# AndyWu0719/Audio-CALM

Measured on NVIDIA B200. Metric: log-mel audio-hours/sec, higher is better.
Workload: dtype f32

## Files before the change

### audio-calm_b200/csrc/acb_kernels.cu

```cuda
#include "audiocalm_b200.h"
#include "acb_fft32.cuh"

#include <cuda_bf16.h>
#include <cuda_runtime.h>

#include <algorithm>
#include <cmath>
#include <cstdio>
#include <cstring>
#include <mutex>
#include <numeric>
#include <string>
#include <vector>

#if !defined(ACB_DEV) || !defined(ACB_ABLATE)
#undef ACB_ABLATE
#define ACB_ABLATE 0
#endif

#ifndef ACB_WIN_FUSE
#define ACB_WIN_FUSE 1
#endif
#ifndef ACB_WIN_T
#define ACB_WIN_T 1
// ... 18 lines not shown
constexpr int kMaxWeights = 4096;
constexpr int kOutStageOffset = 2 * kBins;
static_assert(kScratchFloats % 32 == 8 && kScratchFloats % 4 == 0, "pair stride must be 8 (mod 32) words and 16-byte aligned");
static_assert(kOutStageOffset + kTileFrames * (kMaxMels | 1) <= kScratchFloats, "staged tile must fit above the power spectrum");

thread_local std::string g_last_error;

int fail(int code, const std::string& msg) {
    g_last_error = msg;
    return code;
}
static int cuda_fail(cudaError_t e, const char* what) {
    g_last_error = std::string(what) + ": " + cudaGetErrorString(e);
    return ACB_ERR_CUDA;
}
#define ACB_CUDA(call)                                  \
    do {                                                \
        cudaError_t e__ = (call);                       \
        if (e__ != cudaSuccess) return cuda_fail(e__, #call); \
    } while (0)

__device__ __forceinline__ unsigned smem_addr(const void* p) { return static_cast<unsigned>(__cvta_generic_to_shared(p)); }
__device__ __forceinline__ void mbar_init(unsigned long long* bar, unsigned count) {
    asm volatile("mbarrier.init.shared::cta.b64 [%0], %1;" ::"r"(smem_addr(bar)), "r"(count) : "memory");
}
__device__ __forceinline__ void mbar_arrive(unsigned long long* bar) {
    asm volatile("mbarrier.arrive.shared::cta.b64 _, [%0];" ::"r"(smem_addr(bar)) : "memory");
}
__device__ __forceinline__ void mbar_arrive_expect_tx(unsigned long long* bar, unsigned bytes) {
    asm volatile("mbarrier.arrive.expect_tx.shared::cta.b64 _, [%0], %1;" ::"r"(smem_addr(bar)), "r"(bytes) : "memory");
}
__device__ __forceinline__ bool mbar_wait(unsigned long long* bar, unsigned parity) {
    unsigned ok = 0;
    for (int spin = 0; spin < (1 << 26) && !ok; ++spin) {
        asm volatile("{\n\t.reg .pred p;\n\tmbarrier.try_wait.parity.shared::cta.b64 p, [%1], %2;\n\tselp.u32 %0, 1, 0, p;\n\t}\n"
                     : "=r"(ok) : "r"(smem_addr(bar)), "r"(parity) : "memory");
    }
    return ok != 0;
}
__device__ __forceinline__ void bulk_copy_g2s(void* smem, const void* gmem, unsigned bytes, unsigned long long* bar) {
    asm volatile("cp.async.bulk.shared::cluster.global.mbarrier::complete_tx::bytes [%0], [%1], %2, [%3];"
                 ::"r"(smem_addr(smem)), "l"(gmem), "r"(bytes), "r"(smem_addr(bar)) : "memory");
}

struct LogmelParams {
    const float* window;
    const float4* twiddle;
    const float* plan_w;
    const int* plan_woff;
    const short* plan_trip;
    const short* plan_band;
    const short* plan_astart;
    int n_plan_w;
    int n_mels;
    float clamp_min;
    float log_scale;
    float log_floor;
    const float* wav;
    const long long* clip_offset;
    const long long* clip_length;
    long long clip_stride;
    long long uniform_length;
    const int* tile_start;
    int n_clips;
    int n_tiles;
    int uniform_tiles_per_clip;
    const float* clip_peak;
    void* out;
    int out_bf16;
    int time_major;
    const long long* out_offset;
    long long out_clip_stride;
    long long frame_capacity;
    const long long* frame_capacity_per_clip;
    int pad_multiple;
    int fill_tail;
    float fill_value;
    int affine;
    float affine_mean;
    float affine_inv_std;
    const float* bin_mean;
    const float* bin_std;
    double* moments_partial;
    int* error_flag;
};

struct SmemLayout {
    int samples, scratch, twiddle, window, plan_w, affine, plan_rec, mbar, moments, total_bytes;
};

__host__ __device__ inline int out_row_stride(int n_mels) { return n_mels | 1; }

__host__ __device__ inline SmemLayout make_smem_layout(int kGroups, int n_mels, int n_plan_w, bool with_moments = false) {
    SmemLayout L;
    int off = 0;
    L.samples = off; off += kGroups * kTileSamples;
    L.scratch = off; off += kGroups * kGroupWarps * kScratchFloats;
    L.twiddle = off; off += 5 * 32 * 4;
    L.window = off; off += 32 * 20;
    if (!with_moments) {
        L.plan_rec = off; off += kGroupWarps * kMaxRounds * kSlots * 4;
        L.mbar = off; off += 2 * kGroups;
        off = (off + 3) & ~3;
        L.affine = off; off += 2 * kMaxMels;
        L.plan_w = off; off += (n_plan_w + 3) & ~3;
        L.moments = off;
// ... 194 lines not shown
        const int lane = tid & 31, warp = tid >> 5;
        for (int b = warp; b < n_mels; b += kGroupWarps) fill_span<OutT>(out + (size_t)b * c.cap + f_begin, n_fill, fv, lane, 32);
    }
}

__device__ __forceinline__ float lg2_normal(float x) {
    float y;
    asm("lg2.approx.ftz.f32 %0, %1;" : "=f"(y) : "f"(x));
    return y;
}

__device__ __forceinline__ void two_sum_add(float2& acc, float x) {
    const float t = __fadd_rn(acc.x, x);
    const float bb = __fsub_rn(t, acc.x);
    const float e = __fadd_rn(__fsub_rn(acc.x, __fsub_rn(t, bb)), __fsub_rn(x, bb));
    acc.y = __fadd_rn(acc.y, e);
    acc.x = t;
}

template <int G, bool kMoments, typename OutT>
__global__ void __launch_bounds__(G * kGroupThreads, G == 4 ? 1 : 2) logmel_fused_kernel(const LogmelParams p) {
    constexpr int kGroups = G;
    constexpr int kThreads = G * kGroupThreads;
    extern __shared__ __align__(16) float smem[];
    const SmemLayout L = make_smem_layout(G, p.n_mels, p.n_plan_w, kMoments);
    const int tid = threadIdx.x;
    const int lane = tid & 31;
    const int grp = tid / kGroupThreads;
    const int gt = tid % kGroupThreads;
    const int gw = gt >> 5;
    const int n_mels = p.n_mels;
    const int S = out_row_stride(n_mels);
    const bool write_out = p.out != nullptr;

    float* s_samples = smem + L.samples + grp * kTileSamples;
    float* s_scratch = smem + L.scratch + grp * kGroupWarps * kScratchFloats;
    float* s_out = s_scratch + kOutStageOffset;
    float4* s_tw4 = reinterpret_cast<float4*>(smem + L.twiddle);
    float* s_win = smem + L.window;
    float* s_pw = smem + L.plan_w;
    float2* s_aff = reinterpret_cast<float2*>(smem + L.affine);
    int4* s_rec = reinterpret_cast<int4*>(smem + L.plan_rec);
    float2* s_mom = reinterpret_cast<float2*>(smem + L.moments) + grp * 2 * n_mels;
    unsigned long long* s_full = reinterpret_cast<unsigned long long*>(smem + L.mbar) + grp;

    for (int i = tid; i < 5 * 32; i += kThreads) s_tw4[i] = p.twiddle[i];
    for (int i = tid; i < kNfft / 2; i += kThreads) {
        if (ACB_WIN_T) s_win[(i & 31) * 20 + (i >> 5)] = p.window[i];
        else s_win[i] = p.window[i];
    }
    for (int i = tid; i < p.n_plan_w; i += kThreads) s_pw[i] = p.plan_w[i];
    for (int i = tid; i < kGroupWarps * kMaxRounds * kSlots; i += kThreads) {
        const int slot = i / kSlots, qq = i - slot * kSlots;
        s_rec[i] = make_int4(p.plan_astart[i] >> 1, (p.plan_woff[slot] >> 1) + qq, p.plan_band[i], p.plan_trip[slot]);
    }
    for (int i = tid; i < n_mels; i += kThreads) {
        float sc = 1.f, sh = 0.f;
        if (p.affine == 1) { sc = p.affine_inv_std; sh = -p.affine_mean * p.affine_inv_std; }
        else if (p.affine == 2) { sc = 1.f / __ldg(p.bin_std + i); sh = -__ldg(p.bin_mean + i) * sc; }
        s_aff[i] = make_float2(sc, sh);
    }
    if (kMoments)
        for (int i = gt; i < 2 * n_mels; i += kGroupThreads) s_mom[i] = make_float2(0.f, 0.f);
    if (gt == 0) {
        mbar_init(s_full, 1);
        asm volatile("fence.mbarrier_init.release.cluster;" ::: "memory");
    }
    __syncthreads();

    const long long n_groups = (long long)gridDim.x * kGroups, g_index = (long long)blockIdx.x * kGroups + grp;
    const long long t_begin = (long long)p.n_tiles * g_index / n_groups;
    const long long t_end = (long long)p.n_tiles * (g_index + 1) / n_groups;

    ClipCursor cur;
    bool staged = false;
    unsigned full_parity = 0;
    if (t_begin < t_end) {
        cursor_init(p, cur, t_begin);
        staged = cur.tile_in_clip * kTileFrames < cur.frames;
        if (staged) load_tile_samples(p, cur, s_samples, gt, grp, s_full);
    }

    const int q = lane >> 2;
    const int pl = lane & 3;
    const float* pair_scratch = s_scratch + pl * kScratchFloats;
    float* scr = s_scratch + gw * kScratchFloats;
    float2* scr2 = reinterpret_cast<float2*>(scr);

    for (long long tile = t_begin; tile < t_end; ++tile) {
        if (staged) {
            if (!mbar_wait(s_full, full_parity) && lane == 0) atomicExch(p.error_flag, 1);
            full_parity ^= 1;
        }

        const int f0 = cur.tile_in_clip * kTileFrames;
        const bool has_frames = f0 < cur.frames;
        const bool active = has_frames && f0 + 2 * gw < cur.frames && ACB_ABLATE != 7;

        if (active) {
            float2 pr[16], pi[16];
            {
                const float* sp = s_samples + (2 * gw) * kHop + lane;
                float2 v[20];
#pragma unroll
                for (int r = 0; r < 20; ++r) v[r] = make_float2(sp[32 * (2 * r)], sp[32 * (2 * r + 1)]);
                float4 w4[4];
                if (ACB_WIN_T) {
// ... 56 lines not shown
            __syncwarp();
            {
                const float4* re4 = reinterpret_cast<const float4*>(scr + lane * kRowStride);
                const float4* im4 = reinterpret_cast<const float4*>(scr + kPlaneFloats + lane * kRowStride);
#pragma unroll
                for (int h = 0; h < 8; ++h) {
                    const float4 zr = re4[h], zi = im4[h];
                    pr[brev3(h)] = make_float2(zr.x, zr.y);
                    pr[brev3(h) + 8] = make_float2(zr.z, zr.w);
                    pi[brev3(h)] = make_float2(zi.x, zi.y);
                    pi[brev3(h) + 8] = make_float2(zi.z, zi.w);
                }
            }
            __syncwarp();
            fft32_packed(pr, pi);
            const int src_lane = (32 - lane) & 31;
#pragma unroll
            for (int m = 0; m < 16; ++m) {
                const float alt_r = (m == 0) ? pr[0].x : pr[16 - m].y;
                const float alt_i = (m == 0) ? pi[0].x : pi[16 - m].y;
                const float offer_r = (lane == 0) ? alt_r : pr[15 - m].y;
                const float offer_i = (lane == 0) ? alt_i : pi[15 - m].y;
                const float c = __shfl_sync(0xffffffffu, offer_r, src_lane);
                const float d = __shfl_sync(0xffffffffu, offer_i, src_lane);
                const float a = pr[m].x, b = pi[m].x;
                const float apc = a + c, bmd = b - d, amc = a - c, bpd = b + d;
                const float pa = fmaf(apc, apc, bmd * bmd);
                const float pb = fmaf(amc, amc, bpd * bpd);
                scr2[lane + 32 * m] = make_float2(pa, pb);
            }
        }
        else {
            group_sync(grp);
        }
        const int4* my_rec = s_rec + (gw * kMaxRounds) * kSlots + q;
        int4 rec_next = my_rec[0];
        group_sync(grp);

        ClipCursor nxt = cur;
        staged = false;
        if (tile + 1 < t_end) {
            cursor_advance(p, nxt);
            staged = nxt.tile_in_clip * kTileFrames < nxt.frames;
            if (staged) load_tile_samples(p, nxt, s_samples, gt, grp, s_full);
        }

        const int pad = cur.frames_padded - cur.frames;
        const bool direct = !p.time_major && (f0 + kTileFrames - 1 <= cur.frames - 2 - pad);

        if (has_frames && ACB_ABLATE != 8) {
            const int fA = f0 + 2 * pl;
            OutT* out_clip = reinterpret_cast<OutT*>(p.out) + cur.out_base;
            const bool pair_store = ((cur.cap & 1) == 0) && ((reinterpret_cast<uintptr_t>(out_clip) & (2 * sizeof(OutT) - 1)) == 0);
            for (int r = 0; r < kMaxRounds; ++r) {
                const int4 rec = rec_next;
                const int trip = rec.w;
                if (trip == 0) break;
                if (r + 1 < kMaxRounds) rec_next = my_rec[(r + 1) * kSlots];
                const int b = rec.z;
                const float2 af = s_aff[b < 0 ? 0 : b];
                const float4* p4 = reinterpret_cast<const float4*>(pair_scratch) + rec.x;
                const float2* w2 = reinterpret_cast<const float2*>(s_pw) + rec.y;
                float acc0 = 0.f, acc1 = 0.f, acc2 = 0.f, acc3 = 0.f;
                const int half_trip = ACB_ABLATE == 4 ? 0 : (trip >> 1);
#pragma unroll 4
                for (int i = 0; i < half_trip; ++i) {
                    const float4 pw = p4[i];
                    const float2 w = w2[kSlots * i];
                    acc0 = fmaf(w.x, pw.x, acc0);
                    acc1 = fmaf(w.x, pw.y, acc1);
                    acc2 = fmaf(w.y, pw.z, acc2);
                    acc3 = fmaf(w.y, pw.w, acc3);
                }
                const float mA = (acc0 + acc2) * cur.gain, mB = (acc1 + acc3) * cur.gain;
                float vA = (mA > p.clamp_min) ? lg2_normal(mA) * p.log_scale : p.log_floor;
                float vB = (mB > p.clamp_min) ? lg2_normal(mB) * p.log_scale : p.log_floor;
                if (kMoments) {
                    float s = 0.f, s2 = 0.f;
                    if (b >= 0 && fA < cur.frames) {
                        const float c = (fA <= cur.frames - 2 && fA > cur.frames - 2 - pad) ? 2.f : 1.f;
                        s = c * vA;
                        s2 = s * vA;
                    }
                    if (b >= 0 && fA + 1 < cur.frames) {
                        const float c = (fA + 1 <= cur.frames - 2 && fA + 1 > cur.frames - 2 - pad) ? 2.f : 1.f;
                        const float cv = c * vB;
                        s += cv;
                        s2 = fmaf(cv, vB, s2);
                    }
                    const bool upper = (pl & 2) != 0;
                    float keep = (upper ? s2 : s) + __shfl_xor_sync(0xffffffffu, upper ? s : s2, 2);
                    keep += __shfl_xor_sync(0xffffffffu, keep, 1);
                    if ((pl & 1) == 0 && b >= 0)
                        two_sum_add(s_mom[(upper ? n_mels : 0) + b], keep);
                }
                if (b >= 0) {
                    vA = fmaf(vA, af.x, af.y);
                    vB = fmaf(vB, af.x, af.y);
                    if (direct) {
                        if (write_out) {
                            OutT* dst = out_clip + (size_t)((unsigned)b * (unsigned)cur.cap) + fA;
                            if (pair_store) {
                                store_pair<OutT>(dst, vA, vB);
                            } else {
                                dst[0] = to_out<OutT>(vA);
                                dst[1] = to_out<OutT>(vB);
                            }
                        }
                    } else {
                        s_out[(2 * pl) * S + b] = vA;
                        s_out[(2 * pl + 1) * S + b] = vB;
                    }
                }
            }
        }
        if (!direct) {
            group_sync(grp);
            if (write_out) {
                store_tile<OutT>(p, cur, s_out, n_mels, S, gt);
                if (p.fill_tail && p.tile_start != nullptr && cur.tile_in_clip == cur.tiles_in_clip - 1) fill_row_tail<OutT>(p, cur, n_mels, gt);
            }
        }
        cur = nxt;
    }

    if (kMoments) {
        group_sync(grp);
// ... 358 lines not shown
                                                            long long out_frames, float pad_value,
                                                            const long long* __restrict__ mask_start, const long long* __restrict__ mask_len) {
    constexpr int kT = 64;
    __shared__ float tile[kT][kT + 1];
    const int clip = blockIdx.z;
    const long long t0 = (long long)blockIdx.x * kT;
    const int d0 = blockIdx.y * kT;
    const long long n = lens[clip];
    const T* src = feat + row_offset[clip] * dim;
    const long long m0 = mask_start ? mask_start[clip] : 0, m1 = mask_start ? m0 + mask_len[clip] : 0;
    const int q = threadIdx.x & 15, r0 = threadIdx.x >> 4;
    const bool vec_in = sizeof(T) == 4 && (dim & 3) == 0 && (reinterpret_cast<uintptr_t>(src) & 15) == 0;
#pragma unroll
    for (int pass = 0; pass < kT / 16; ++pass) {
        const int r = pass * 16 + r0;
        const long long t = t0 + r;
        const int d = d0 + 4 * q;
        float v[4] = {pad_value, pad_value, pad_value, pad_value};
        if (t < n) {
            const bool masked = t >= m0 && t < m1;
            if (vec_in && d + 3 < dim) {
                if constexpr (sizeof(T) == 4) {
                    const float4 u = __ldg(reinterpret_cast<const float4*>(src + t * dim + d));
                    v[0] = u.x; v[1] = u.y; v[2] = u.z; v[3] = u.w;
                }
            } else {
#pragma unroll
                for (int j = 0; j < 4; ++j) if (d + j < dim) v[j] = (float)src[t * dim + d + j];
            }
            if (masked) { v[0] = v[1] = v[2] = v[3] = 0.f; }
        }
#pragma unroll
        for (int j = 0; j < 4; ++j) tile[4 * q + j][r] = v[j];
    }
    __syncthreads();
    const bool vec_out = sizeof(T) == 4 && (out_frames & 3) == 0 && (reinterpret_cast<uintptr_t>(out) & 15) == 0;
#pragma unroll
    for (int pass = 0; pass < kT / 16; ++pass) {
        const int r = pass * 16 + r0;
        const int d = d0 + r;
        const long long t = t0 + 4 * q;
        if (d >= dim || t >= out_frames) continue;
        T* dst = out + ((long long)clip * dim + d) * out_frames + t;
        if (vec_out && t + 3 < out_frames) {
            if constexpr (sizeof(T) == 4)
                *reinterpret_cast<float4*>(dst) = make_float4(tile[r][4 * q], tile[r][4 * q + 1], tile[r][4 * q + 2], tile[r][4 * q + 3]);
        } else {
#pragma unroll
            for (int j = 0; j < 4; ++j) if (t + j < out_frames) dst[j] = from_float<T>(tile[r][4 * q + j]);
        }
    }
}

}

struct acb_frontend {
    int device = 0;
    int n_fft = 0, hop = 0, n_mels = 0, n_weights = 0, log_kind = 0;
    float clamp_min = 0.f;
    int num_sms = 0;
    int groups = 0;
    int grid = 0;
    int smem_bytes = 0;
    int smem_bytes_moments = 0;
    void* d_blob = nullptr;
    const float* d_window = nullptr;
    const float4* d_twiddle = nullptr;
    const float* d_plan_w = nullptr;
    const int* d_plan_woff = nullptr;
    const short* d_plan_trip = nullptr;
    const short* d_plan_band = nullptr;
    const short* d_plan_astart = nullptr;
    int n_plan_w = 0;
    int* d_err = nullptr;
    cudaStream_t s_in = nullptr, s_out = nullptr;
    std::vector<cudaEvent_t> ev;
    std::mutex mu;
};

using namespace acb;

extern "C" {

int acb_abi_version(void) { return ACB_ABI_VERSION; }
const char* acb_last_error(void) { return g_last_error.c_str(); }
int acb_frames_per_tile(void) { return kTileFrames; }

int64_t acb_frames_for_length(int64_t length, int n_fft, int hop) {
    if (n_fft <= 0 || hop <= 0) return -1;
    if (length <= n_fft / 2) return -1;
    return 1 + length / hop;
}

int64_t acb_padded_frames(int64_t frames, int multiple) {
    if (multiple <= 1) return frames;
    const int64_t r = frames % multiple;
    return r ? frames + (multiple - r) : frames;
}

int64_t acb_plan_tiles(const int64_t* lengths_host, int32_t n_clips, int n_fft, int hop, int64_t frame_capacity,
                       int32_t* tile_start_host) {
    if (!lengths_host || !tile_start_host || n_clips < 0) return fail(ACB_ERR_INVALID, "acb_plan_tiles: null argument");
    int64_t total = 0;
    for (int32_t i = 0; i < n_clips; ++i) {
        const int64_t T = acb_frames_for_length(lengths_host[i], n_fft, hop);
        if (T < 0) {
            return fail(ACB_ERR_INVALID, "acb_plan_tiles: clip " + std::to_string(i) + " has " + std::to_string(lengths_host[i]) +
                                             " samples; reflect padding needs more than " + std::to_string(n_fft / 2));
        }
        const int64_t cover = frame_capacity > 0 ? frame_capacity : T;
        tile_start_host[i] = (int32_t)total;
        total += (cover + kTileFrames - 1) / kTileFrames;
        if (total > INT32_MAX) return fail(ACB_ERR_INVALID, "acb_plan_tiles: more than 2^31 tiles in one call");
    }
    tile_start_host[n_clips] = (int32_t)total;
    return total;
}

int acb_frontend_create(acb_frontend** out, int device, int n_fft, int hop, int n_mels, const float* window_host,
                        const float* fb_host, float clamp_min, int log_kind) {
    if (!out || !window_host || !fb_host) return fail(ACB_ERR_INVALID, "acb_frontend_create: null argument");
    if (n_fft != kNfft || hop != kHop)
        return fail(ACB_ERR_UNSUPPORTED, "acb_frontend_create: this build has kernels for n_fft=1024, hop=256 only (got n_fft=" +
                                             std::to_string(n_fft) + ", hop=" + std::to_string(hop) + ")");
    if (n_mels < 1 || n_mels > kMaxMels) return fail(ACB_ERR_UNSUPPORTED, "acb_frontend_create: n_mels must be in [1, 128]");
    if (log_kind != ACB_LOG_NATURAL && log_kind != ACB_LOG_10) return fail(ACB_ERR_INVALID, "acb_frontend_create: bad log_kind");
    if (!(clamp_min >= 1.17549435e-38f)) return fail(ACB_ERR_INVALID, "acb_frontend_create: clamp_min must be a positive normal float");
    for (int n = 0; n < kNfft / 2; ++n) {
        const double dev = std::fabs((double)window_host[n + kNfft / 2] - (1.0 - (double)window_host[n]));
        if (!(dev <= 1e-6))
            return fail(ACB_ERR_UNSUPPORTED, "acb_frontend_create: the window must have the periodic-Hann property w[n + 512] = 1 - w[n] "
                                             "(deviation " + std::to_string(dev) + " at n=" + std::to_string(n) + ")");
    }
    const int n_freq = n_fft / 2 + 1;

    std::vector<int> start(n_mels, 0), len(n_mels, 0), off(n_mels, 0);
    std::vector<float> weights;
    for (int m = 0; m < n_mels; ++m) {
        int lo = -1, hi = -1;
        for (int f = 0; f < n_freq; ++f)
            if (fb_host[(size_t)f * n_mels + m] != 0.f) { if (lo < 0) lo = f; hi = f; }
        off[m] = (int)weights.size();
        if (lo >= 0) {
            if (hi >= kBins) {
                if (fb_host[(size_t)(n_freq - 1) * n_mels + m] != 0.f)
                    return fail(ACB_ERR_UNSUPPORTED, "acb_frontend_create: filterbank has weight on the Nyquist bin");
            }
            start[m] = lo;
            len[m] = hi - lo + 1;
            for (int f = lo; f <= hi; ++f) weights.push_back(fb_host[(size_t)f * n_mels + m] * 0.25f);
        }
    }
    if ((int)weights.size() > kMaxWeights) return fail(ACB_ERR_UNSUPPORTED, "acb_frontend_create: filterbank too dense");

    std::vector<int> alen(n_mels), aend(n_mels);
    for (int m = 0; m < n_mels; ++m) {
        if (len[m] == 0) { start[m] = 0; len[m] = 0; }
        aend[m] = (start[m] + std::max(len[m], 1) + 1) & ~1;
        alen[m] = aend[m] - (start[m] & ~1);
    }
    std::vector<int> order(n_mels);
    std::iota(order.begin(), order.end(), 0);
    std::stable_sort(order.begin(), order.end(), [&](int a, int b) { return alen[a] > alen[b]; });
    const int n_rounds = (n_mels + kSlots - 1) / kSlots;
    std::vector<short> plan_band(kGroupWarps * kMaxRounds * kSlots, (short)-1), plan_astart(kGroupWarps * kMaxRounds * kSlots, (short)0),
        plan_trip(kGroupWarps * kMaxRounds, (short)0);
    std::vector<int> plan_woff(kGroupWarps * kMaxRounds, 0);
    std::vector<float> plan_w;
    std::vector<int> load(kGroupWarps, 0), rounds(kGroupWarps, 0);
    for (int g = 0; g < n_rounds; ++g) {
        int best = -1;
        for (int w = 0; w < kGroupWarps; ++w)
            if (rounds[w] < kMaxRounds && (best < 0 || load[w] < load[best])) best = w;
        if (best < 0) return fail(ACB_ERR_UNSUPPORTED, "acb_frontend_create: mel plan overflow");
        std::vector<int> par[2];
        for (int q = 0; q < kSlots && kSlots * g + q < n_mels; ++q) {
            const int m = order[kSlots * g + q];
            par[((start[m] & ~1) >> 1) & 1].push_back(m);
        }
        std::vector<int> slots;
        while (!par[0].empty() && !par[1].empty()) {
            slots.push_back(par[0].back()); par[0].pop_back();
            slots.push_back(par[1].back()); par[1].pop_back();
        }
        for (int k = 0; k < 2; ++k)
            for (int m : par[k]) slots.push_back(m);
        std::vector<int> shift(slots.size(), 0), as(slots.size(), 0);
        int trip = 2;
        for (int iter = 0; iter < 8; ++iter) {
            trip = 2;
            for (size_t i = 0; i < slots.size(); ++i) trip = std::max(trip, aend[slots[i]] - ((start[slots[i]] & ~1) - shift[i]));
            for (size_t i = 0; i < slots.size(); ++i) {
                as[i] = (start[slots[i]] & ~1) - shift[i];
                if (as[i] + trip > kBins) as[i] = std::max(0, (kBins - trip) & ~1);
            }
            bool changed = false;
            for (size_t i = 0; i + 1 < slots.size(); i += 2) {
                if ((((as[i] >> 1) ^ (as[i + 1] >> 1)) & 1) != 0) continue;
                const size_t x = (as[i + 1] >= 2 && (start[slots[i + 1]] & ~1) - shift[i + 1] == as[i + 1]) ? i + 1
                                 : ((as[i] >= 2 && (start[slots[i]] & ~1) - shift[i] == as[i]) ? i : slots.size());
                if (x < slots.size()) { shift[x] += 2; changed = true; }
            }
            if (!changed) break;
        }
        const int slot = best * kMaxRounds + rounds[best];
        plan_trip[slot] = (short)trip;
        plan_woff[slot] = (int)plan_w.size();
        plan_w.resize(plan_w.size() + (size_t)trip * kSlots, 0.f);
        float* wbase = plan_w.data() + plan_woff[slot];
        for (size_t q = 0; q < slots.size(); ++q) {
            const int m = slots[q];
            plan_band[slot * kSlots + q] = (short)m;
            plan_astart[slot * kSlots + q] = (short)as[q];
            for (int i = 0; i < len[m]; ++i) {
                const int rel = start[m] + i - as[q];
                if (rel < 0 || rel >= trip) return fail(ACB_ERR_UNSUPPORTED, "acb_frontend_create: mel plan window error");
                wbase[(rel >> 1) * (2 * kSlots) + q * 2 + (rel & 1)] = weights[off[m] + i];
            }
        }
        load[best] += trip + 16;
        rounds[best]++;
    }
    if ((int)plan_w.size() > kMaxWeights * 4) return fail(ACB_ERR_UNSUPPORTED, "acb_frontend_create: mel plan too large");

    std::vector<float4> tw(5 * 32);
    for (int l = 0; l < 32; ++l) {
        auto wre = [&](int m) { return (float)cos(-2.0 * M_PI * (double)(m * l) / 1024.0); };
        auto wim = [&](int m) { return (float)sin(-2.0 * M_PI * (double)(m * l) / 1024.0); };
        for (int k = 0; k < 4; ++k) tw[k * 32 + l] = make_float4(wre(k), wre(k + 16), wim(k), wim(k + 16));
        tw[4 * 32 + l] = make_float4(wre(4), wim(4), 0.f, 0.f);
    }

    int prev = 0;
    ACB_CUDA(cudaGetDevice(&prev));
    ACB_CUDA(cudaSetDevice(device));
    auto* fe = new acb_frontend();
    fe->device = device; fe->n_fft = n_fft; fe->hop = hop; fe->n_mels = n_mels; fe->n_weights = (int)weights.size();
    fe->n_plan_w = (int)plan_w.size();
    fe->log_kind = log_kind; fe->clamp_min = clamp_min;

    size_t o = 0;
    auto take = [&](size_t bytes) { size_t r = o; o += (bytes + 255) & ~size_t(255); return r; };
    const size_t o_win = take(sizeof(float) * kNfft), o_tw = take(sizeof(float4) * 160),
                 o_pw = take(sizeof(float) * std::max<size_t>(plan_w.size(), 1)), o_po = take(sizeof(int) * plan_woff.size()),
                 o_pt = take(sizeof(short) * plan_trip.size()), o_pb = take(sizeof(short) * plan_band.size()),
                 o_pa = take(sizeof(short) * plan_astart.size()), o_err = take(16);
    std::vector<unsigned char> host(o, 0);
    memcpy(host.data() + o_win, window_host, sizeof(float) * kNfft);
    memcpy(host.data() + o_tw, tw.data(), sizeof(float4) * 160);
    if (!plan_w.empty()) memcpy(host.data() + o_pw, plan_w.data(), sizeof(float) * plan_w.size());
    memcpy(host.data() + o_po, plan_woff.data(), sizeof(int) * plan_woff.size());
    memcpy(host.data() + o_pt, plan_trip.data(), sizeof(short) * plan_trip.size());
    memcpy(host.data() + o_pb, plan_band.data(), sizeof(short) * plan_band.size());
    memcpy(host.data() + o_pa, plan_astart.data(), sizeof(short) * plan_astart.size());
    cudaError_t e = cudaMalloc(&fe->d_blob, o);
    if (e == cudaSuccess) e = cudaMemcpy(fe->d_blob, host.data(), o, cudaMemcpyHostToDevice);
    cudaDeviceProp prop;
    if (e == cudaSuccess) e = cudaGetDeviceProperties(&prop, device);
    const int optin = (int)prop.sharedMemPerBlockOptin;
    fe->groups = std::max(make_smem_layout(kMaxGroups, n_mels, fe->n_plan_w, true).total_bytes,
                          make_smem_layout(kMaxGroups, n_mels, fe->n_plan_w, false).total_bytes) <= optin ? kMaxGroups : 2;
    const SmemLayout L = make_smem_layout(fe->groups, n_mels, fe->n_plan_w, false);
    const SmemLayout Lm = make_smem_layout(fe->groups, n_mels, fe->n_plan_w, true);
    fe->smem_bytes = L.total_bytes;
    fe->smem_bytes_moments = Lm.total_bytes;
    if (e == cudaSuccess && std::max(L.total_bytes, Lm.total_bytes) > optin) {
        if (fe->d_blob) cudaFree(fe->d_blob);
        delete fe;
        cudaSetDevice(prev);
        return fail(ACB_ERR_UNSUPPORTED, "acb_frontend_create: filterbank plan needs more shared memory than the device offers");
    }
    int occ = 0;
    auto prepare = [&](auto kernel, int threads) {
        if (e == cudaSuccess) e = cudaFuncSetAttribute(kernel, cudaFuncAttributeMaxDynamicSharedMemorySize, optin);
        if (e == cudaSuccess && occ == 0) e = cudaOccupancyMaxActiveBlocksPerMultiprocessor(&occ, kernel, threads, L.total_bytes);
    };
    if (fe->groups == 4) {
        prepare(logmel_fused_kernel<4, false, float>, 4 * kGroupThreads);
        prepare(logmel_fused_kernel<4, false, __nv_bfloat16>, 4 * kGroupThreads);
        prepare(logmel_fused_kernel<4, true, float>, 4 * kGroupThreads);
        prepare(logmel_fused_kernel<4, true, __nv_bfloat16>, 4 * kGroupThreads);
    } else {
        prepare(logmel_fused_kernel<2, false, float>, 2 * kGroupThreads);
        prepare(logmel_fused_kernel<2, false, __nv_bfloat16>, 2 * kGroupThreads);
        prepare(logmel_fused_kernel<2, true, float>, 2 * kGroupThreads);
        prepare(logmel_fused_kernel<2, true, __nv_bfloat16>, 2 * kGroupThreads);
    }
    if (e != cudaSuccess) {
        if (fe->d_blob) cudaFree(fe->d_blob);
        delete fe;
        cudaSetDevice(prev);
// ... 5 lines not shown
    fe->d_window = reinterpret_cast<const float*>(base + o_win);
    fe->d_twiddle = reinterpret_cast<const float4*>(base + o_tw);
    fe->d_plan_w = reinterpret_cast<const float*>(base + o_pw);
    fe->d_plan_woff = reinterpret_cast<const int*>(base + o_po);
    fe->d_plan_trip = reinterpret_cast<const short*>(base + o_pt);
    fe->d_plan_band = reinterpret_cast<const short*>(base + o_pb);
    fe->d_plan_astart = reinterpret_cast<const short*>(base + o_pa);
    fe->d_err = reinterpret_cast<int*>(base + o_err);
    cudaSetDevice(prev);
    *out = fe;
    return ACB_OK;
}

int acb_frontend_destroy(acb_frontend* fe) {
    if (!fe) return ACB_OK;
    int prev = 0;
    cudaGetDevice(&prev);
    cudaSetDevice(fe->device);
    for (auto ev : fe->ev) cudaEventDestroy(ev);
    if (fe->s_in) cudaStreamDestroy(fe->s_in);
    if (fe->s_out) cudaStreamDestroy(fe->s_out);
    if (fe->d_blob) cudaFree(fe->d_blob);
    cudaSetDevice(prev);
    delete fe;
    return ACB_OK;
}

int64_t acb_moments_workspace_bytes(const acb_frontend* fe) {
    if (!fe) return fail(ACB_ERR_INVALID, "acb_moments_workspace_bytes: null handle");
    return (int64_t)fe->grid * fe->groups * 2 * fe->n_mels * (int64_t)sizeof(double);
}

int acb_logmel_forward(const acb_frontend* fe, const acb_logmel_args* a, void* stream) {
    if (!fe || !a) return fail(ACB_ERR_INVALID, "acb_logmel_forward: null argument");
    if (a->n_clips <= 0 || a->n_tiles <= 0) return ACB_OK;
    if (!a->wav) return fail(ACB_ERR_INVALID, "acb_logmel_forward: null wav");
    if (!a->out && !a->moments) return fail(ACB_ERR_INVALID, "acb_logmel_forward: out may be NULL only for a statistics-only launch (moments set)");
    if (a->out_dtype != ACB_F32 && a->out_dtype != ACB_BF16) return fail(ACB_ERR_INVALID, "acb_logmel_forward: bad out_dtype");
    if (a->out_layout != ACB_MEL_MAJOR && a->out_layout != ACB_TIME_MAJOR) return fail(ACB_ERR_INVALID, "acb_logmel_forward: bad out_layout");
    if (a->pad_multiple < 1) return fail(ACB_ERR_INVALID, "acb_logmel_forward: pad_multiple must be >= 1");
    if (kTileFrames % a->pad_multiple != 0)
        return fail(ACB_ERR_UNSUPPORTED, "acb_logmel_forward: pad_multiple must divide the " + std::to_string(kTileFrames) + "-frame tile (1, 2, 4 or 8)");
    if (a->affine < 0 || a->affine > 2) return fail(ACB_ERR_INVALID, "acb_logmel_forward: bad affine mode");
    if (a->affine == 2 && (!a->bin_mean || !a->bin_std)) return fail(ACB_ERR_INVALID, "acb_logmel_forward: per-bin affine needs bin_mean/bin_std");
    if (a->affine == 1 && !(a->affine_std > 0.f)) return fail(ACB_ERR_INVALID, "acb_logmel_forward: affine_std must be > 0");
    if (a->moments && !a->moments_workspace) return fail(ACB_ERR_INVALID, "acb_logmel_forward: moments need a workspace");
    if (!a->frame_capacity_per_clip && a->frame_capacity <= 0) return fail(ACB_ERR_INVALID, "acb_logmel_forward: frame_capacity must be > 0");
    if (a->frame_capacity * (int64_t)fe->n_mels >= (int64_t)1 << 32) return fail(ACB_ERR_INVALID, "acb_logmel_forward: n_mels * frame_capacity must be < 2^32");

    LogmelParams p{};
    p.window = fe->d_window; p.twiddle = fe->d_twiddle;
    p.plan_w = fe->d_plan_w; p.plan_woff = fe->d_plan_woff; p.plan_trip = fe->d_plan_trip;
    p.plan_band = fe->d_plan_band; p.plan_astart = fe->d_plan_astart; p.n_plan_w = fe->n_plan_w;
    p.n_mels = fe->n_mels; p.clamp_min = fe->clamp_min;
    p.log_scale = fe->log_kind == ACB_LOG_10 ? 0.30102999566398120f : 0.69314718055994531f;
    p.log_floor = fe->log_kind == ACB_LOG_10 ? log10f(fe->clamp_min) : logf(fe->clamp_min);
    p.wav = a->wav;
    p.clip_offset = reinterpret_cast<const long long*>(a->clip_offset);
    p.clip_length = reinterpret_cast<const long long*>(a->clip_length);
    p.clip_stride = a->clip_stride; p.uniform_length = a->uniform_length;
    p.tile_start = a->tile_start; p.n_clips = a->n_clips; p.n_tiles = a->n_tiles;
    p.uniform_tiles_per_clip = 1;
    if (!a->tile_start && a->clip_length) {
        if (!a->fill_tail || a->frame_capacity_per_clip)
            return fail(ACB_ERR_INVALID, "acb_logmel_forward: ragged clips need tile_start (acb_plan_tiles) unless fill_tail pads every clip to frame_capacity");
        p.uniform_tiles_per_clip = (int)((a->frame_capacity + kTileFrames - 1) / kTileFrames);
        if ((int64_t)p.uniform_tiles_per_clip * a->n_clips != a->n_tiles)
            return fail(ACB_ERR_INVALID, "acb_logmel_forward: n_tiles does not match n_clips * tiles per clip");
    } else if (!a->tile_start) {
        const int64_t T = acb_frames_for_length(a->uniform_length, fe->n_fft, fe->hop);
        if (T < 0) return fail(ACB_ERR_INVALID, "acb_logmel_forward: clips of " + std::to_string(a->uniform_length) +
                                                    " samples are too short for reflect padding of " + std::to_string(fe->n_fft / 2));
        const int64_t cover = a->fill_tail ? a->frame_capacity : T;
        p.uniform_tiles_per_clip = (int)((cover + kTileFrames - 1) / kTileFrames);
        if ((int64_t)p.uniform_tiles_per_clip * a->n_clips != a->n_tiles)
            return fail(ACB_ERR_INVALID, "acb_logmel_forward: n_tiles does not match n_clips * tiles per clip");
        if (acb_padded_frames(T, a->pad_multiple) > a->frame_capacity)
            return fail(ACB_ERR_INVALID, "acb_logmel_forward: frame_capacity smaller than the padded frame count");
        if (acb_padded_frames(T, a->pad_multiple) - T >= T)
            return fail(ACB_ERR_INVALID, "acb_logmel_forward: reflect pad to the multiple needs more frames than the clip has");
    }
    p.clip_peak = a->clip_peak;
    p.out = a->out; p.out_bf16 = a->out_dtype == ACB_BF16; p.time_major = a->out_layout == ACB_TIME_MAJOR;
    p.out_offset = reinterpret_cast<const long long*>(a->out_offset);
    p.out_clip_stride = a->out_clip_stride; p.frame_capacity = a->frame_capacity;
    p.frame_capacity_per_clip = reinterpret_cast<const long long*>(a->frame_capacity_per_clip);
    p.pad_multiple = a->pad_multiple; p.fill_tail = a->fill_tail; p.fill_value = a->fill_value;
    p.affine = a->affine; p.affine_mean = a->affine_mean;
    p.affine_inv_std = a->affine == 1 ? (float)(1.0 / (double)a->affine_std) : 1.f;
    p.bin_mean = a->bin_mean; p.bin_std = a->bin_std;
    p.moments_partial = a->moments ? static_cast<double*>(a->moments_workspace) : nullptr;
    p.error_flag = fe->d_err;

    int prev = 0;
    ACB_CUDA(cudaGetDevice(&prev));
    if (prev != fe->device) ACB_CUDA(cudaSetDevice(fe->device));
    cudaStream_t st = static_cast<cudaStream_t>(stream);
    const int grid = fe->grid;
    const int threads = fe->groups * kGroupThreads;
    const size_t smem = a->moments ? fe->smem_bytes_moments : fe->smem_bytes;
    auto launch = [&](auto kernel) { kernel<<<grid, threads, smem, st>>>(p); };
    if (fe->groups == 4) {
        if (a->moments) { if (p.out_bf16) launch(logmel_fused_kernel<4, true, __nv_bfloat16>); else launch(logmel_fused_kernel<4, true, float>); }
        else { if (p.out_bf16) launch(logmel_fused_kernel<4, false, __nv_bfloat16>); else launch(logmel_fused_kernel<4, false, float>); }
    } else {
        if (a->moments) { if (p.out_bf16) launch(logmel_fused_kernel<2, true, __nv_bfloat16>); else launch(logmel_fused_kernel<2, true, float>); }
// ... 305 lines not shown
```

Before: 4590.

## Compute mel filterbank via shared segment partials instead of per-band dot products

Adds a segment-based mel plan for triangular filterbanks whose bands overlap only with their neighbours. Each power bin is multiplied once into two adjacent-band accumulators per segment, and partial sums are passed to the next slot with a warp shuffle plus a carry across rounds. This roughly halves the redundant reads of overlapping bins compared with the per-band plan. It falls back to the old band plan when the structure doesn't fit, and adds a dynamic-programming host planner, a debug export, and float4 weight loads with extra shuffles per round.

```diff
diff --git a/audio-calm_b200/csrc/acb_kernels.cu b/audio-calm_b200/csrc/acb_kernels.cu
--- a/audio-calm_b200/csrc/acb_kernels.cu
+++ b/audio-calm_b200/csrc/acb_kernels.cu
@@ -94,6 +94,7 @@
     const short* plan_band;
     const short* plan_astart;
     int n_plan_w;
+    int mel_segments;
     int n_mels;
     float clamp_min;
     float log_scale;
@@ -394,7 +395,8 @@
     for (int i = tid; i < p.n_plan_w; i += kThreads) s_pw[i] = p.plan_w[i];
     for (int i = tid; i < kGroupWarps * kMaxRounds * kSlots; i += kThreads) {
         const int slot = i / kSlots, qq = i - slot * kSlots;
-        s_rec[i] = make_int4(p.plan_astart[i] >> 1, (p.plan_woff[slot] >> 1) + qq, p.plan_band[i], p.plan_trip[slot]);
+        const int woff = p.plan_woff[slot];
+        s_rec[i] = make_int4(p.plan_astart[i] >> 1, (p.mel_segments ? woff >> 2 : woff >> 1) + qq, p.plan_band[i], p.plan_trip[slot]);
     }
     for (int i = tid; i < n_mels; i += kThreads) {
         float sc = 1.f, sh = 0.f;
@@ -557,6 +559,7 @@
             const int fA = f0 + 2 * pl;
             OutT* out_clip = reinterpret_cast<OutT*>(p.out) + cur.out_base;
             const bool pair_store = ((cur.cap & 1) == 0) && ((reinterpret_cast<uintptr_t>(out_clip) & (2 * sizeof(OutT) - 1)) == 0);
+            float carry_a = 0.f, carry_b = 0.f;
             for (int r = 0; r < kMaxRounds; ++r) {
                 const int4 rec = rec_next;
                 const int trip = rec.w;
@@ -565,19 +568,44 @@
                 const int b = rec.z;
                 const float2 af = s_aff[b < 0 ? 0 : b];
                 const float4* p4 = reinterpret_cast<const float4*>(pair_scratch) + rec.x;
-                const float2* w2 = reinterpret_cast<const float2*>(s_pw) + rec.y;
+                const int half_trip = ACB_ABLATE == 4 ? 0 : (trip >> 1);
                 float acc0 = 0.f, acc1 = 0.f, acc2 = 0.f, acc3 = 0.f;
-                const int half_trip = ACB_ABLATE == 4 ? 0 : (trip >> 1);
+                float mA, mB;
+                if (p.mel_segments) {
+                    const float4* w4 = reinterpret_cast<const float4*>(s_pw) + rec.y;
 #pragma unroll 4
-                for (int i = 0; i < half_trip; ++i) {
-                    const float4 pw = p4[i];
-                    const float2 w = w2[kSlots * i];
-                    acc0 = fmaf(w.x, pw.x, acc0);
-                    acc1 = fmaf(w.x, pw.y, acc1);
-                    acc2 = fmaf(w.y, pw.z, acc2);
-                    acc3 = fmaf(w.y, pw.w, acc3);
+                    for (int i = 0; i < half_trip; ++i) {
+                        const float4 pw = p4[i];
+                        const float4 w = w4[kSlots * i];
+                        acc0 = fmaf(w.x, pw.x, acc0);
+                        acc1 = fmaf(w.x, pw.y, acc1);
+                        acc2 = fmaf(w.y, pw.x, acc2);
+                        acc3 = fmaf(w.y, pw.y, acc3);
+                        acc0 = fmaf(w.z, pw.z, acc0);
+                        acc1 = fmaf(w.z, pw.w, acc1);
+                        acc2 = fmaf(w.w, pw.z, acc2);
+                        acc3 = fmaf(w.w, pw.w, acc3);
+                    }
+                    const int prev_slot = (lane + 32 - 4) & 31;
+                    const float tA = __shfl_sync(0xffffffffu, acc2, prev_slot), tB = __shfl_sync(0xffffffffu, acc3, prev_slot);
+                    mA = (acc0 + (q == 0 ? carry_a : tA)) * cur.gain;
+                    mB = (acc1 + (q == 0 ? carry_b : tB)) * cur.gain;
+                    carry_a = tA;
+                    carry_b = tB;
+                } else {
+                    const float2* w2 = reinterpret_cast<const float2*>(s_pw) + rec.y;
+#pragma unroll 4
+                    for (int i = 0; i < half_trip; ++i) {
+                        const float4 pw = p4[i];
+                        const float2 w = w2[kSlots * i];
+                        acc0 = fmaf(w.x, pw.x, acc0);
+                        acc1 = fmaf(w.x, pw.y, acc1);
+                        acc2 = fmaf(w.y, pw.z, acc2);
+                        acc3 = fmaf(w.y, pw.w, acc3);
+                    }
+                    mA = (acc0 + acc2) * cur.gain;
+                    mB = (acc1 + acc3) * cur.gain;
                 }
-                const float mA = (acc0 + acc2) * cur.gain, mB = (acc1 + acc3) * cur.gain;
                 float vA = (mA > p.clamp_min) ? lg2_normal(mA) * p.log_scale : p.log_floor;
                 float vB = (mB > p.clamp_min) ? lg2_normal(mB) * p.log_scale : p.log_floor;
                 if (kMoments) {
@@ -1042,6 +1070,246 @@
     }
 }
 
+struct MelPlan {
+    bool segments = false;
+    std::vector<short> band = std::vector<short>(kGroupWarps * kMaxRounds * kSlots, (short)-1);
+    std::vector<short> astart = std::vector<short>(kGroupWarps * kMaxRounds * kSlots, (short)0);
+    std::vector<short> trip = std::vector<short>(kGroupWarps * kMaxRounds, (short)0);
+    std::vector<int> woff = std::vector<int>(kGroupWarps * kMaxRounds, 0);
+    std::vector<float> w;
+    int n_weights = 0;
+};
+
+struct BandedBank {
+    std::vector<int> start, len, off;
+    std::vector<float> weights;
+};
+
+static int build_band_plan(int n_mels, BandedBank bd, MelPlan& P) {
+    std::vector<int>& start = bd.start;
+    std::vector<int>& len = bd.len;
+    std::vector<short>& plan_band = P.band;
+    std::vector<short>& plan_astart = P.astart;
+    std::vector<short>& plan_trip = P.trip;
+    std::vector<int>& plan_woff = P.woff;
+    std::vector<float>& plan_w = P.w;
+    std::vector<int> alen(n_mels), aend(n_mels);
+    for (int m = 0; m < n_mels; ++m) {
+        if (len[m] == 0) { start[m] = 0; len[m] = 0; }
+        aend[m] = (start[m] + std::max(len[m], 1) + 1) & ~1;
+        alen[m] = aend[m] - (start[m] & ~1);
+    }
+    std::vector<int> order(n_mels);
+    std::iota(order.begin(), order.end(), 0);
+    std::stable_sort(order.begin(), order.end(), [&](int a, int b) { return alen[a] > alen[b]; });
+    const int n_rounds = (n_mels + kSlots - 1) / kSlots;
+    std::vector<int> load(kGroupWarps, 0), rounds(kGroupWarps, 0);
+    for (int g = 0; g < n_rounds; ++g) {
+        int best = -1;
+        for (int w = 0; w < kGroupWarps; ++w)
+            if (rounds[w] < kMaxRounds && (best < 0 || load[w] < load[best])) best = w;
+        if (best < 0) return fail(ACB_ERR_UNSUPPORTED, "acb_frontend_create: mel plan overflow");
+        std::vector<int> par[2];
+        for (int q = 0; q < kSlots && kSlots * g + q < n_mels; ++q) {
+            const int m = order[kSlots * g + q];
+            par[((start[m] & ~1) >> 1) & 1].push_back(m);
+        }
+        std::vector<int> slots;
+        while (!par[0].empty() && !par[1].empty()) {
+            slots.push_back(par[0].back()); par[0].pop_back();
+            slots.push_back(par[1].back()); par[1].pop_back();
+        }
+        for (int k = 0; k < 2; ++k)
+            for (int m : par[k]) slots.push_back(m);
+        std::vector<int> shift(slots.size(), 0), as(slots.size(), 0);
+        int trip = 2;
+        for (int iter = 0; iter < 8; ++iter) {
+            trip = 2;
+            for (size_t i = 0; i < slots.size(); ++i) trip = std::max(trip, aend[slots[i]] - ((start[slots[i]] & ~1) - shift[i]));
+            for (size_t i = 0; i < slots.size(); ++i) {
+                as[i] = (start[slots[i]] & ~1) - shift[i];
+                if (as[i] + trip > kBins) as[i] = std::max(0, (kBins - trip) & ~1);
+            }
+            bool changed = false;
+            for (size_t i = 0; i + 1 < slots.size(); i += 2) {
+                if ((((as[i] >> 1) ^ (as[i + 1] >> 1)) & 1) != 0) continue;
+                const size_t x = (as[i + 1] >= 2 && (start[slots[i + 1]] & ~1) - shift[i + 1] == as[i + 1]) ? i + 1
+                                 : ((as[i] >= 2 && (start[slots[i]] & ~1) - shift[i] == as[i]) ? i : slots.size());
+                if (x < slots.size()) { shift[x] += 2; changed = true; }
+            }
+            if (!changed) break;
+        }
+        const int slot = best * kMaxRounds + rounds[best];
+        plan_trip[slot] = (short)trip;
+        plan_woff[slot] = (int)plan_w.size();
+        plan_w.resize(plan_w.size() + (size_t)trip * kSlots, 0.f);
+        float* wbase = plan_w.data() + plan_woff[slot];
+        for (size_t q = 0; q < slots.size(); ++q) {
+            const int m = slots[q];
+            plan_band[slot * kSlots + q] = (short)m;
+            plan_astart[slot * kSlots + q] = (short)as[q];
+            for (int i = 0; i < len[m]; ++i) {
+                const int rel = start[m] + i - as[q];
+                if (rel < 0 || rel >= trip) return fail(ACB_ERR_UNSUPPORTED, "acb_frontend_create: mel plan window error");
+                wbase[(rel >> 1) * (2 * kSlots) + q * 2 + (rel & 1)] = bd.weights[bd.off[m] + i];
+            }
+        }
+        load[best] += trip + 16;
+        rounds[best]++;
+    }
+    return ACB_OK;
+}
+
+static bool build_segment_plan(int n_mels, const BandedBank& bd, MelPlan& P) {
+    const int M = n_mels;
+    for (int m = 0; m < M; ++m)
+        if (bd.len[m] == 0) return false;
+    std::vector<int> o(M);
+    std::iota(o.begin(), o.end(), 0);
+    std::stable_sort(o.begin(), o.end(), [&](int a, int b) { return bd.start[a] < bd.start[b]; });
+    auto s = [&](int k) { return bd.start[o[k]]; };
+    auto e = [&](int k) { return bd.start[o[k]] + bd.len[o[k]] - 1; };
+    for (int k = 1; k < M; ++k)
+        if (s(k) <= s(k - 1)) return false;
+    for (int k = 1; k + 1 < M; ++k)
+        if (e(k - 1) >= s(k + 1)) return false;
+    std::vector<int> lo(M + 2);
+    for (int k = 0; k < M; ++k) lo[k] = s(k);
+    const int end_prev = M >= 2 ? e(M - 2) + 1 : lo[M - 1];
+    lo[M + 1] = std::max(e(M - 1) + 1, end_prev);
+    lo[M] = std::min(std::max(end_prev, lo[M - 1]), lo[M + 1]);
+    auto wt = [&](int k, int seg, int f) -> float {
+        if (k < 0 || k >= M || f < lo[seg] || f >= lo[seg + 1]) return 0.f;
+        const int m = o[k], r = f - bd.start[m];
+        return (r >= 0 && r < bd.len[m]) ? bd.weights[bd.off[m] + r] : 0.f;
+    };
+    std::vector<int> ext_a((M + 1) * 4, kBins), ext_z((M + 1) * 4, 0);
+    for (int k = 0; k <= M; ++k)
+        for (int kind = 1; kind < 4; ++kind)
+            for (int f = lo[k]; f < lo[k + 1]; ++f)
+                if (((kind & 1) && wt(k - 1, k, f) != 0.f) || ((kind & 2) && wt(k, k, f) != 0.f)) {
+                    ext_a[k * 4 + kind] = std::min(ext_a[k * 4 + kind], f);
+                    ext_z[k * 4 + kind] = f + 1;
+                }
+    auto kind_of = [](int B0, int B1, int k) { return (k > B0 ? 1 : 0) | (k < B1 ? 2 : 0); };
+    auto solve_round = [&](int B0, int B1, int k0, int n, short* first) -> int {
+        int a[kSlots], z[kSlots], trip = 2;
+        for (int q = 0; q < kSlots; ++q) {
+            a[q] = kBins; z[q] = 0;
+            if (q < n) { const int i = (k0 + q) * 4 + kind_of(B0, B1, k0 + q); a[q] = ext_a[i]; z[q] = ext_z[i]; }
+            if (z[q] > a[q]) trip = std::max(trip, (z[q] - (a[q] & ~1) + 1) & ~1);
+        }
+        for (; trip <= kBins; trip += 2) {
+            bool ok = true;
+            for (int h = 0; h < kSlots && ok; h += 2) {
+                int used[2], n_used = 0;
+                for (int q = h; q < h + 2; ++q)
+                    if (z[q] > a[q]) used[n_used++] = q;
+                for (int par = 0; par < 2; ++par) {
+                    ok = true;
+                    for (int j = 0; j < n_used && ok; ++j) {
+                        const int q = used[j], top = std::min(a[q], kBins - trip) & ~1, want = par ^ j;
+                        const int x = top - 2 * (((top >> 1) ^ want) & 1);
+                        ok = x >= 0 && x + trip >= z[q];
+                        first[q] = (short)x;
+                    }
+                    if (ok) break;
+                }
+                for (int q = h; q < h + 2 && ok; ++q)
+                    if (!(z[q] > a[q])) first[q] = n_used ? first[used[0]] : 0;
+            }
+            if (ok) return trip;
+        }
+        return 0;
+    };
+    constexpr int kWarpSlots = kMaxRounds * kSlots;
+    auto warp_cost = [&](int B0, int B1) -> int {
+        if (B0 == B1) return 0;
+        const int n = B1 - B0 + 1;
+        if (n > kWarpSlots) return -1;
+        int cost = 0;
+        short first[kSlots];
+        for (int k0 = B0; k0 <= B1; k0 += kSlots) {
+            const int trip = solve_round(B0, B1, k0, std::min(kSlots, B1 + 1 - k0), first);
+            if (trip == 0) return -1;
+            cost += trip + 16;
+        }
+        return cost;
+    };
+    using Load = std::pair<int, int>;
+    const Load kNone(INT32_MAX, INT32_MAX);
+    std::vector<std::vector<Load>> best(kGroupWarps + 1, std::vector<Load>(M + 1, kNone));
+    std::vector<std::vector<int>> cut(kGroupWarps + 1, std::vector<int>(M + 1, -1));
+    best[0][0] = Load(0, 0);
+    for (int j = 0; j <= M; ++j)
+        for (int i = std::max(0, j - kWarpSlots + 1); i <= j; ++i) {
+            const int c = warp_cost(i, j);
+            if (c < 0) continue;
+            for (int w = 1; w <= kGroupWarps; ++w) {
+                if (best[w - 1][i] == kNone) continue;
+                const Load l(std::max(best[w - 1][i].first, c), best[w - 1][i].second + c);
+                if (l < best[w][j]) { best[w][j] = l; cut[w][j] = i; }
+            }
+        }
+    if (best[kGroupWarps][M] == kNone) return false;
+    int B1 = M;
+    for (int w = kGroupWarps - 1; w >= 0; --w) {
+        const int B0 = cut[w + 1][B1];
+        for (int k0 = B0, r = 0; B0 < B1 && k0 <= B1; k0 += kSlots, ++r) {
+            const int slot = w * kMaxRounds + r, n = std::min(kSlots, B1 + 1 - k0);
+            short* first = P.astart.data() + slot * kSlots;
+            const int trip = solve_round(B0, B1, k0, n, first);
+            P.trip[slot] = (short)trip;
+            P.woff[slot] = (int)P.w.size();
+            P.w.resize(P.w.size() + (size_t)trip * kSlots * 2, 0.f);
+            float* wbase = P.w.data() + P.woff[slot];
+            for (int q = 0; q < n; ++q) {
+                const int k = k0 + q, kind = kind_of(B0, B1, k);
+                P.band[slot * kSlots + q] = (short)(k > B0 ? o[k - 1] : -1);
+                for (int i = 0; i < trip; ++i) {
+                    const int f = first[q] + i;
+                    float* wq = wbase + ((i >> 1) * kSlots + q) * 4 + (i & 1) * 2;
+                    wq[0] = (kind & 1) ? wt(k - 1, k, f) : 0.f;
+                    wq[1] = (kind & 2) ? wt(k, k, f) : 0.f;
+                }
+            }
+        }
+        B1 = B0;
+    }
+    P.segments = true;
+    return true;
+}
+
+static int build_mel_plan(int n_mels, const float* fb_host, MelPlan& P) {
+    const int n_freq = kNfft / 2 + 1;
+    BandedBank bd;
+    bd.start.assign(n_mels, 0); bd.len.assign(n_mels, 0); bd.off.assign(n_mels, 0);
+    for (int m = 0; m < n_mels; ++m) {
+        int lo = -1, hi = -1;
+        for (int f = 0; f < n_freq; ++f)
+            if (fb_host[(size_t)f * n_mels + m] != 0.f) { if (lo < 0) lo = f; hi = f; }
+        bd.off[m] = (int)bd.weights.size();
+        if (lo >= 0) {
+            if (hi >= kBins) {
+                if (fb_host[(size_t)(n_freq - 1) * n_mels + m] != 0.f)
+                    return fail(ACB_ERR_UNSUPPORTED, "acb_frontend_create: filterbank has weight on the Nyquist bin");
+            }
+            bd.start[m] = lo;
+            bd.len[m] = hi - lo + 1;
+            for (int f = lo; f <= hi; ++f) bd.weights.push_back(fb_host[(size_t)f * n_mels + m] * 0.25f);
+        }
+    }
+    if ((int)bd.weights.size() > kMaxWeights) return fail(ACB_ERR_UNSUPPORTED, "acb_frontend_create: filterbank too dense");
+    P.n_weights = (int)bd.weights.size();
+    if (!build_segment_plan(n_mels, bd, P) || (int)P.w.size() > kMaxWeights * 4) {
+        P = MelPlan();
+        P.n_weights = (int)bd.weights.size();
+        if (const int rc = build_band_plan(n_mels, bd, P)) return rc;
+    }
+    if ((int)P.w.size() > kMaxWeights * 4) return fail(ACB_ERR_UNSUPPORTED, "acb_frontend_create: mel plan too large");
+    return ACB_OK;
+}
+
 }
 
 struct acb_frontend {
@@ -1062,6 +1330,7 @@
     const short* d_plan_band = nullptr;
     const short* d_plan_astart = nullptr;
     int n_plan_w = 0;
+    bool mel_segments = false;
     int* d_err = nullptr;
     cudaStream_t s_in = nullptr, s_out = nullptr;
     std::vector<cudaEvent_t> ev;
@@ -1105,6 +1374,22 @@
     }
     tile_start_host[n_clips] = (int32_t)total;
     return total;
+}
+
+int acb_debug_mel_plan(int n_mels, const float* fb_host, int* segments, short* band, short* astart, short* trip, int* woff,
+                       float* w, int w_cap) {
+    if (!fb_host || !segments || !band || !astart || !trip || !woff || (!w && w_cap > 0))
+        return fail(ACB_ERR_INVALID, "acb_debug_mel_plan: null argument");
+    if (n_mels < 1 || n_mels > kMaxMels) return fail(ACB_ERR_UNSUPPORTED, "acb_debug_mel_plan: n_mels must be in [1, 128]");
+    MelPlan plan;
+    if (const int rc = build_mel_plan(n_mels, fb_host, plan)) return rc;
+    *segments = plan.segments ? 1 : 0;
+    std::copy(plan.band.begin(), plan.band.end(), band);
+    std::copy(plan.astart.begin(), plan.astart.end(), astart);
+    std::copy(plan.trip.begin(), plan.trip.end(), trip);
+    std::copy(plan.woff.begin(), plan.woff.end(), woff);
+    std::copy_n(plan.w.begin(), std::min<size_t>(plan.w.size(), (size_t)std::max(w_cap, 0)), w);
+    return (int)plan.w.size();
 }
 
 int acb_frontend_create(acb_frontend** out, int device, int n_fft, int hop, int n_mels, const float* window_host,
@@ -1122,96 +1407,13 @@
             return fail(ACB_ERR_UNSUPPORTED, "acb_frontend_create: the window must have the periodic-Hann property w[n + 512] = 1 - w[n] "
                                              "(deviation " + std::to_string(dev) + " at n=" + std::to_string(n) + ")");
     }
-    const int n_freq = n_fft / 2 + 1;
-
-    std::vector<int> start(n_mels, 0), len(n_mels, 0), off(n_mels, 0);
-    std::vector<float> weights;
-    for (int m = 0; m < n_mels; ++m) {
-        int lo = -1, hi = -1;
-        for (int f = 0; f < n_freq; ++f)
-            if (fb_host[(size_t)f * n_mels + m] != 0.f) { if (lo < 0) lo = f; hi = f; }
-        off[m] = (int)weights.size();
-        if (lo >= 0) {
-            if (hi >= kBins) {
-                if (fb_host[(size_t)(n_freq - 1) * n_mels + m] != 0.f)
-                    return fail(ACB_ERR_UNSUPPORTED, "acb_frontend_create: filterbank has weight on the Nyquist bin");
-            }
-            start[m] = lo;
-            len[m] = hi - lo + 1;
-            for (int f = lo; f <= hi; ++f) weights.push_back(fb_host[(size_t)f * n_mels + m] * 0.25f);
-        }
-    }
-    if ((int)weights.size() > kMaxWeights) return fail(ACB_ERR_UNSUPPORTED, "acb_frontend_create: filterbank too dense");
-
-    std::vector<int> alen(n_mels), aend(n_mels);
-    for (int m = 0; m < n_mels; ++m) {
-        if (len[m] == 0) { start[m] = 0; len[m] = 0; }
-        aend[m] = (start[m] + std::max(len[m], 1) + 1) & ~1;
-        alen[m] = aend[m] - (start[m] & ~1);
-    }
-    std::vector<int> order(n_mels);
-    std::iota(order.begin(), order.end(), 0);
-    std::stable_sort(order.begin(), order.end(), [&](int a, int b) { return alen[a] > alen[b]; });
-    const int n_rounds = (n_mels + kSlots - 1) / kSlots;
-    std::vector<short> plan_band(kGroupWarps * kMaxRounds * kSlots, (short)-1), plan_astart(kGroupWarps * kMaxRounds * kSlots, (short)0),
-        plan_trip(kGroupWarps * kMaxRounds, (short)0);
-    std::vector<int> plan_woff(kGroupWarps * kMaxRounds, 0);
-    std::vector<float> plan_w;
-    std::vector<int> load(kGroupWarps, 0), rounds(kGroupWarps, 0);
-    for (int g = 0; g < n_rounds; ++g) {
-        int best = -1;
-        for (int w = 0; w < kGroupWarps; ++w)
-            if (rounds[w] < kMaxRounds && (best < 0 || load[w] < load[best])) best = w;
-        if (best < 0) return fail(ACB_ERR_UNSUPPORTED, "acb_frontend_create: mel plan overflow");
-        std::vector<int> par[2];
-        for (int q = 0; q < kSlots && kSlots * g + q < n_mels; ++q) {
-            const int m = order[kSlots * g + q];
-            par[((start[m] & ~1) >> 1) & 1].push_back(m);
-        }
-        std::vector<int> slots;
-        while (!par[0].empty() && !par[1].empty()) {
-            slots.push_back(par[0].back()); par[0].pop_back();
-            slots.push_back(par[1].back()); par[1].pop_back();
-        }
-        for (int k = 0; k < 2; ++k)
-            for (int m : par[k]) slots.push_back(m);
-        std::vector<int> shift(slots.size(), 0), as(slots.size(), 0);
-        int trip = 2;
-        for (int iter = 0; iter < 8; ++iter) {
-            trip = 2;
-            for (size_t i = 0; i < slots.size(); ++i) trip = std::max(trip, aend[slots[i]] - ((start[slots[i]] & ~1) - shift[i]));
-            for (size_t i = 0; i < slots.size(); ++i) {
-                as[i] = (start[slots[i]] & ~1) - shift[i];
-                if (as[i] + trip > kBins) as[i] = std::max(0, (kBins - trip) & ~1);
-            }
-            bool changed = false;
-            for (size_t i = 0; i + 1 < slots.size(); i += 2) {
-                if ((((as[i] >> 1) ^ (as[i + 1] >> 1)) & 1) != 0) continue;
-                const size_t x = (as[i + 1] >= 2 && (start[slots[i + 1]] & ~1) - shift[i + 1] == as[i + 1]) ? i + 1
-                                 : ((as[i] >= 2 && (start[slots[i]] & ~1) - shift[i] == as[i]) ? i : slots.size());
-                if (x < slots.size()) { shift[x] += 2; changed = true; }
-            }
-            if (!changed) break;
-        }
-        const int slot = best * kMaxRounds + rounds[best];
-        plan_trip[slot] = (short)trip;
-        plan_woff[slot] = (int)plan_w.size();
-        plan_w.resize(plan_w.size() + (size_t)trip * kSlots, 0.f);
-        float* wbase = plan_w.data() + plan_woff[slot];
-        for (size_t q = 0; q < slots.size(); ++q) {
-            const int m = slots[q];
-            plan_band[slot * kSlots + q] = (short)m;
-            plan_astart[slot * kSlots + q] = (short)as[q];
-            for (int i = 0; i < len[m]; ++i) {
-                const int rel = start[m] + i - as[q];
-                if (rel < 0 || rel >= trip) return fail(ACB_ERR_UNSUPPORTED, "acb_frontend_create: mel plan window error");
-                wbase[(rel >> 1) * (2 * kSlots) + q * 2 + (rel & 1)] = weights[off[m] + i];
-            }
-        }
-        load[best] += trip + 16;
-        rounds[best]++;
-    }
-    if ((int)plan_w.size() > kMaxWeights * 4) return fail(ACB_ERR_UNSUPPORTED, "acb_frontend_create: mel plan too large");
+    MelPlan plan;
+    if (const int rc = build_mel_plan(n_mels, fb_host, plan)) return rc;
+    const std::vector<float>& plan_w = plan.w;
+    const std::vector<int>& plan_woff = plan.woff;
+    const std::vector<short>& plan_trip = plan.trip;
+    const std::vector<short>& plan_band = plan.band;
+    const std::vector<short>& plan_astart = plan.astart;
 
     std::vector<float4> tw(5 * 32);
     for (int l = 0; l < 32; ++l) {
@@ -1225,8 +1427,9 @@
     ACB_CUDA(cudaGetDevice(&prev));
     ACB_CUDA(cudaSetDevice(device));
     auto* fe = new acb_frontend();
-    fe->device = device; fe->n_fft = n_fft; fe->hop = hop; fe->n_mels = n_mels; fe->n_weights = (int)weights.size();
+    fe->device = device; fe->n_fft = n_fft; fe->hop = hop; fe->n_mels = n_mels; fe->n_weights = plan.n_weights;
     fe->n_plan_w = (int)plan_w.size();
+    fe->mel_segments = plan.segments;
     fe->log_kind = log_kind; fe->clamp_min = clamp_min;
 
     size_t o = 0;
@@ -1338,6 +1541,7 @@
     p.window = fe->d_window; p.twiddle = fe->d_twiddle;
     p.plan_w = fe->d_plan_w; p.plan_woff = fe->d_plan_woff; p.plan_trip = fe->d_plan_trip;
     p.plan_band = fe->d_plan_band; p.plan_astart = fe->d_plan_astart; p.n_plan_w = fe->n_plan_w;
+    p.mel_segments = fe->mel_segments;
     p.n_mels = fe->n_mels; p.clamp_min = fe->clamp_min;
     p.log_scale = fe->log_kind == ACB_LOG_10 ? 0.30102999566398120f : 0.69314718055994531f;
     p.log_floor = fe->log_kind == ACB_LOG_10 ? log10f(fe->clamp_min) : logf(fe->clamp_min);
```

Result: slower. 4527, median of 6 (-1.4%).
